# geneo4PETSc/geneo4PETSc

Measured on AMD Instinct MI355X. Metric: GenEO-PCG setup+solve sec and SpMV GB/s, 3D Laplacian 50M DoF, 1/2/4/8 GPUs, higher is better.
Workload: dtype f64

## Files before the change

geneo4petsc_amd/csrc/backend.h:

```cpp
#pragma once
#include <cstddef>
#include <cstdint>

namespace bk {

const char* name();
void set_stream(void* hip_stream);
void* get_stream();
void sync();
void side_stream_begin(void* after = nullptr, bool use_after = false);
void side_stream_end();

int   device_count();
int   set_device(int ordinal);
int   current_device();
int   thread_device_check();
void* alloc(size_t bytes);
void  dfree(void* p);
void  alloc_cache_release();
void  mem_info(double* live, double* live_peak, double* footprint_peak, double* cached, double* dev_free, double* dev_total,
               bool reset_peaks);
void  alloc_stats(double* alloc_s, double* free_s, long long* n);
void  h2d(void* d, const void* h, size_t bytes);
void  d2h(void* h, const void* d, size_t bytes);
// ... 67 lines not shown
void spmv_fused_lp(const Csr& a, int epi, const double* x, double* y, const double* b, double* z, const double* dinv, double w);
bool csr_fusable(const Csr& a);
void spmm_fused(const Csr& a, int epi, const double* X, int ldx, double* Y, int ldy, int m, const double* B, int ldb,
                double* Z, int ldz, const double* dinv, double w);
void csr_diag(const Csr& a, double* diag);
int  recip_positive(double* x, int n);

void gather(double* out, const double* in, const int* idx, int n);
void gather_mul(double* out, const double* in, const int* idx, const double* d, int n);
void segsum(double* out, const double* in, const int* ptr, const int* idx, int nseg, bool accumulate);

void gather_rows(double* out, const double* in, const int* idx, int n, int w);
void segsum_rows(double* out, const double* in, const int* ptr, const int* idx, int nseg, int w, bool accumulate);

void set(double* x, double v, int n);
void copy(double* y, const double* x, int n);
void axpy(double* y, double a, const double* x, int n);
void axpby(double* y, double a, const double* x, double b, int n);
void xmy(double* y, const double* x, const double* d, int n);
void axpy_dev(double* y, const double* a_dev, double sign, const double* x, int n);
void dot(const double* x, const double* y, int n, double* out_dev);

constexpr int CHUNK = 1024;
struct Chunks {
  int nchunk = 0, nsub = 0, n = 0;
  int* start = nullptr;
  int* len = nullptr;
  int* sub = nullptr;
  int* subptr = nullptr;
  int* suboff = nullptr;
  double* partial = nullptr;
  double* totals = nullptr;
  int maxsub_chunks = 0;
};
void set_par_reduce_min(int chunks);
int get_par_reduce_min();
Chunks chunks_upload(int nsub, const int* h_suboff );
void   chunks_free(Chunks& c);
void seg_dot(const Chunks& c, const double* x, const double* y, double* out, int stride, int slot);

void cg_start(const Chunks& c, double* sc, double* x, double* r, double* z, double* p, const double* b,
              const double* dinv);
void seg_pap(const Chunks& c, const double* p, const double* q);
void seg_partial(const Chunks& c, const double* x, const double* y, int slot);
void cg_set_rz(const Chunks& c, double* sc);
void dense_sym_apply(const Chunks& c, const double* inv, const int64_t* base, const double* B, int ldb, double* X,
                     int ldx, int m);
void cg_update(const Chunks& c, double* sc, int parity, double* x, double* r, double* z, const double* p,
               const double* q, const double* dinv);
void cg_direction(const Chunks& c, double* sc, int parity, double* p, const double* z, double tol2);

void gram(const Chunks& c, const double* S, int lds, int p, const double* T, int ldt, int q, double* G);
void gram2(const Chunks& c, const double* S1, int lds1, int p1, const double* S2, int lds2, int p2, const double* T, int ldt,
           int q, double* G);
void block_mul(const Chunks& c, const double* S, int lds, int p, const double* C, int q, double* Y, int ldy,
               bool accumulate);
void block_residual(const Chunks& c, const double* AX, int lda, const double* BX, int ldb, const double* lam,
                    int m, double* R, int ldr, double* nrm);
void block_colnorm(const Chunks& c, const double* X, int ldx, int m, double* nrm);
void block_residual_norms(const Chunks& c, const double* AX, int lda, const double* BX, int ldb, const double* lam,
                          int m, double* R, int ldr, const double* colmask, double* nrm3);
void lobpcg_update32(const Chunks& c, const double* S, const double* AS, const double* BS, const double* C,
                     const double* keep, const double* lam, const double* mask, double* T, double* AT, double* BT,
                     double* R);
void lobpcg_update32_basis(const Chunks& c, const double* S, const double* C, const double* keep, double* T);
bool lobpcg_update32_available();
// ... 43 lines not shown
```

geneo4petsc_amd/csrc/backend_hip.hip:

```cpp
#include <hip/hip_runtime.h>

#include <algorithm>
#include <atomic>
#include <cstdio>
#include <cstdlib>
#include <functional>
#include <stdexcept>
#include <string>
#include <chrono>
#include <condition_variable>
#include <cstring>
#include <thread>
#include <type_traits>
#include <map>
#include <mutex>
#include <unordered_map>
#include <vector>

#include "backend.h"

#define HIPCHK(x)                                                                          \
  do {                                                                                     \
    hipError_t e_ = (x);                                                                   \
    if (e_ != hipSuccess) {                                                                \
      throw std::runtime_error(std::string("HIP error ") + hipGetErrorString(e_) + " at " + \
                               __FILE__ + ":" + std::to_string(__LINE__));                 \
    }                                                                                      \
  } while (0)

namespace bk {

static hipStream_t g_stream_main = nullptr;
static thread_local hipStream_t t_stream_side = nullptr;
static thread_local bool t_side = false;
static thread_local bool g_capturing = false;
static thread_local hipStream_t g_capture_stream = nullptr;
static std::atomic<int> g_device{-1};
static thread_local bool t_dev_bound = false;
static inline void bind_thread() {
  if (t_dev_bound) return;
  t_dev_bound = true;
  const int want = g_device.load(std::memory_order_acquire);
  if (want < 0) {
    int d = 0;
    if (hipGetDevice(&d) == hipSuccess) g_device.store(d, std::memory_order_release);
    else (void)hipGetLastError();
  } else {
    int d = -1;
    if (hipGetDevice(&d) != hipSuccess || d != want) {
      if (hipSetDevice(want) != hipSuccess) throw std::runtime_error("geneo: hipSetDevice failed on a library thread");
    }
  }
// ... 1627 lines not shown
};
template <int EPI>
__device__ __forceinline__ double epi_apply(double sum, double e_b, double e_z, double e_d, double e_x, double w,
                                            double& zout) {
  if (EPI == EPI_NONE) {
    return sum;
  } else if (EPI == EPI_RES) {
    return e_b - sum;
  } else if (EPI == EPI_ADD) {
    return e_z + sum;
  } else if (EPI == EPI_JAC) {
    return e_x + w * e_d * (e_b - sum);
  } else if (EPI == EPI_POST) {
    return w * e_d * (e_z + e_b) + sum;
  } else {
    zout = w * e_d * e_b;
    return e_b - w * sum;
  }
}
struct EpiRow {
  double b = 0.0, z = 0.0, d = 0.0, x = 0.0;
};
template <int EPI>
__device__ __forceinline__ EpiRow epi_load_row(int64_t r, const double* __restrict__ b, const double* __restrict__ z,
                                               const double* __restrict__ dinv, const double* __restrict__ x) {
  EpiRow e;
  if (EpiReads<EPI>::b) e.b = b[r];
  if (EpiReads<EPI>::z) e.z = z[r];
  if (EpiReads<EPI>::d(z)) e.d = dinv[r];
  if (EpiReads<EPI>::x) e.x = x[r];
  return e;
}
template <int EPI>
__device__ __forceinline__ void epi_store_row(int64_t r, double sum, const EpiRow& e, double w, double* __restrict__ y,
                                              double* __restrict__ z) {
  double zv = 0.0;
  const double yv = epi_apply<EPI>(sum, e.b, e.z, e.d, e.x, w, zv);
  if (EPI == EPI_PRE && z) z[r] = zv;
  y[r] = yv;
}

template <bool PAIR_SUM, bool NARROW, bool P16, bool EPI_EARLY>
struct SlicePolicy {
  static constexpr bool pair_sum = PAIR_SUM, narrow = NARROW, p16 = P16, epi_early = EPI_EARLY;
  static_assert(NARROW || !P16, "the predicated form continues the narrow forms");
  static __device__ __forceinline__ double sum4(const double (&acc)[4]) {
    return PAIR_SUM ? (acc[0] + acc[1]) + (acc[2] + acc[3]) : ((acc[0] + acc[1]) + acc[2]) + acc[3];
  }
};
typedef SlicePolicy<false, true, false, true> SliceSell;
typedef SlicePolicy<false, false, false, true> SliceEpi;
typedef SlicePolicy<true, false, false, false> SliceWide;
typedef SlicePolicy<true, true, true, true> SliceLp;

template <int KW, typename VT, int EPI, bool NT, typename POL, typename SRC>
__device__ __forceinline__ double row_sum_fixed(const SRC& src, const VT* __restrict__ val, int64_t e0,
                                                const double* __restrict__ xin, const double* __restrict__ cs) {
  int c[KW];
  double v[KW];
#pragma unroll
  for (int u = 0; u < KW; ++u) {
    c[u] = src.at(u, e0);
    v[u] = (double)(NT ? __builtin_nontemporal_load(val + e0 + 64 * u) : val[e0 + 64 * u]);
  }
  src.template finish<KW>(c);
  double xv[KW];
#pragma unroll
  for (int u = 0; u < KW; ++u) xv[u] = (EPI == EPI_PRE && cs) ? xin[c[u]] * cs[c[u]] : xin[c[u]];
  double acc[4] = {0.0, 0.0, 0.0, 0.0};
  constexpr int NG = KW / 4;
#pragma unroll
  for (int g = 0; g < NG; ++g)
// ... 17 lines not shown
    default: return row_sum_fixed<8, VT, EPI, NT, POL>(src, val, e0, xin, cs);
  }
}
template <int EPI, typename COLT, bool NT>
__device__ __forceinline__ double lp_row_sum_p16(const COLT* __restrict__ col, const float* __restrict__ val, int64_t e0,
                                                 int wd, const int4 cb, const double* __restrict__ xin,
                                                 const double* __restrict__ cs) {
  int c[16];
  double v[16];
#pragma unroll
  for (int u = 0; u < 16; ++u) {
    c[u] = cb.x;
    v[u] = 0.0;
    if (u < wd) {
      c[u] = (u < cb.z ? cb.x : cb.y) + (int)(NT ? __builtin_nontemporal_load(col + e0 + 64 * u) : col[e0 + 64 * u]);
      v[u] = (double)(NT ? __builtin_nontemporal_load(val + e0 + 64 * u) : val[e0 + 64 * u]);
    }
  }
  double xv[16];
#pragma unroll
  for (int u = 0; u < 16; ++u) {
    xv[u] = 0.0;
    if (u < wd) xv[u] = (EPI == EPI_PRE && cs) ? xin[c[u]] * cs[c[u]] : xin[c[u]];
  }
  double acc[4] = {0.0, 0.0, 0.0, 0.0};
  const int ng4 = (wd >> 2) << 2;
#pragma unroll
  for (int u = 0; u < 16; ++u) {
    if (u < ng4) acc[u & 3] += v[u] * xv[u];
    else if (u < wd) acc[0] += v[u] * xv[u];
  }
  return (acc[0] + acc[1]) + (acc[2] + acc[3]);
}
template <typename VT, typename COLT, int EPI, int WPS, bool NT, bool OFFS, typename POL>
__device__ __forceinline__ void spmv_sell_slice(const int64_t* __restrict__ sl_ptr, int nslice, int n,
                                                const COLT* __restrict__ col, const VT* __restrict__ val,
                                                const int* __restrict__ base, const double* __restrict__ x,
                                                double* __restrict__ y, const double* __restrict__ b,
                                                double* __restrict__ z, const double* __restrict__ dinv, double w,
                                                const double* __restrict__ cs ,
                                                const unsigned char* __restrict__ omask, const int* __restrict__ orec) {
  static_assert(WPS == 1 || (WPS == 4 && !OFFS), "a coded slice belongs to one wave");
  constexpr bool FIXED = POL::narrow && WPS == 1;
  const int wv = threadIdx.x >> 6, l = threadIdx.x & 63;
  int s;
  if (WPS == 1) {
    const int nwb = (nslice + 3) >> 2;
    const int t = xcd_remap(blockIdx.x, nwb);
    s = 4 * t + wv;
    if (t >= nwb || s >= nslice) return;
  } else {
    s = xcd_remap(blockIdx.x, nslice);
    if (s >= nslice) return;
  }
  const int su = OFFS ? __builtin_amdgcn_readfirstlane(s) : s;
  const int64_t a = sl_ptr[su], e1 = sl_ptr[su + 1];
  const int4 cb = lp_base_of(base, su);
  int4 o0 = int4{OFF_NONE, 0, 0, 0}, o1 = int4{0, 0, 0, 0};
  int nofix = 0;
  if (OFFS) {
    const int4* rec = reinterpret_cast<const int4*>(orec) + 2 * (int64_t)su;
    o0 = rec[0];
    o1 = rec[1];
    nofix = g_lp_no_fixed;
  }
  const double* __restrict__ xin = (EPI == EPI_PRE) ? b : x;
  const int r = 64 * s + l;
  unsigned char om = 0;
  int oov = 0;
  if (OFFS) {
    om = omask[r];
    oov = orec[8 * (int64_t)su + (l & 7)];
  }
  EpiRow ep;
  if (POL::epi_early && r < n && (WPS == 1 || wv == 0)) ep = epi_load_row<EPI>(r, b, z, dinv, x);
  constexpr int STEP = 64 * WPS;
  double acc[4] = {0.0, 0.0, 0.0, 0.0};
  int64_t e = a + (WPS == 1 ? 0 : 64 * wv) + l;
  int k = (WPS == 1 ? 0 : wv);
  const int wd = (int)((e1 - a) >> 6);
  double fixed_sum = 0.0;
  bool fixed = false;
  if constexpr (FIXED) fixed = wd >= 1 && wd <= (POL::p16 ? 16 : 8) && !(OFFS ? nofix : g_lp_no_fixed);
  if constexpr (FIXED) {
    if (OFFS && fixed && o0.x != OFF_NONE) {
      fixed_sum = row_sum_narrow<VT, EPI, NT, POL>(wd, ColsOffset{o0, o1, om, oov, r, r < n ? r : n - 1}, val, e, xin, cs);
      e = e1;
    } else if (POL::p16 && fixed && wd > 8) {
      if constexpr (POL::p16) fixed_sum = lp_row_sum_p16<EPI, COLT, NT>(col, val, e, wd, cb, xin, cs);
      e = e1;
    } else if (fixed) {
      fixed_sum = row_sum_narrow<VT, EPI, NT, POL>(wd, ColsStored<COLT, NT>{col, cb}, val, e, xin, cs);
      e = e1;
    }
  }
  for (; e + STEP * 3 < e1; e += STEP * 4, k += WPS * 4) {
    int c[4];
    double v[4];
#pragma unroll
    for (int u = 0; u < 4; ++u) {
      c[u] = (k + WPS * u < cb.z ? cb.x : cb.y) + (int)(NT ? __builtin_nontemporal_load(col + e + STEP * u) : col[e + STEP * u]);
      v[u] = (double)(NT ? __builtin_nontemporal_load(val + e + STEP * u) : val[e + STEP * u]);
    }
#pragma unroll
    for (int u = 0; u < 4; ++u) acc[u] += v[u] * ((EPI == EPI_PRE && cs) ? xin[c[u]] * cs[c[u]] : xin[c[u]]);
  }
  for (; e < e1; e += STEP, k += WPS) {
    const int c0 = (k < cb.z ? cb.x : cb.y) + (int)(NT ? __builtin_nontemporal_load(col + e) : col[e]);
    const double v0 = (double)(NT ? __builtin_nontemporal_load(val + e) : val[e]);
    acc[0] += v0 * ((EPI == EPI_PRE && cs) ? xin[c0] * cs[c0] : xin[c0]);
  }
  double sum = fixed ? fixed_sum : POL::sum4(acc);
  if (WPS == 4) {
    __shared__ double part[3][64];
    if (wv > 0) part[wv - 1][l] = sum;
    __syncthreads();
    if (wv > 0) return;
    sum = (sum + part[0][l]) + (part[1][l] + part[2][l]);
  }
  if (r >= n) return;
  if (!POL::epi_early) ep = epi_load_row<EPI>(r, b, z, dinv, x);
  epi_store_row<EPI>(r, sum, ep, w, y, z);
}

template <bool NT, typename COLT = int, bool OFFS = false>
__global__ __launch_bounds__(256) void k_spmv_sell(const int64_t* __restrict__ sl_ptr, int nslice, int n,
                                                   const COLT* __restrict__ col, const double* __restrict__ val,
                                                   const double* __restrict__ x, double* __restrict__ y,
                                                   const int* __restrict__ cbase = nullptr,
                                                   const unsigned char* __restrict__ omask = nullptr,
                                                   const int* __restrict__ orec = nullptr) {
  spmv_sell_slice<double, COLT, EPI_NONE, 1, NT, OFFS, SliceSell>(sl_ptr, nslice, n, col, val, cbase, x, y, nullptr, nullptr,
                                                                  nullptr, 0.0, nullptr, omask, orec);
}
template <bool NT, int EPI>
__global__ __launch_bounds__(256) void k_spmv_sell_epi(const int64_t* __restrict__ sl_ptr, int nslice, int n,
                                                       const int* __restrict__ col, const double* __restrict__ val,
                                                       const double* __restrict__ x, double* __restrict__ y,
                                                       const double* __restrict__ b, double* __restrict__ z,
                                                       const double* __restrict__ dinv, double w,
                                                       const double* __restrict__ cs) {
  spmv_sell_slice<double, int, EPI, 1, NT, false, SliceEpi>(sl_ptr, nslice, n, col, val, nullptr, x, y, b, z, dinv, w, cs,
                                                            nullptr, nullptr);
}
template <int EPI>
__global__ __launch_bounds__(256) void k_spmv_sell_wide(const int64_t* __restrict__ sl_ptr, int nslice, int n,
                                                        const int* __restrict__ col, const double* __restrict__ val,
                                                        const double* __restrict__ x, double* __restrict__ y,
                                                        const double* __restrict__ b, double* __restrict__ z,
                                                        const double* __restrict__ dinv, double w,
                                                        const double* __restrict__ cs) {
// ... 309 lines not shown
    d2h(hstat, dstat, sizeof(hstat));
    dfree(dstat);
    int hfail[2];
    memcpy(hfail, &hstat[0], sizeof(hfail));
    const unsigned long long* hcnt = hstat + 1;
    if (hfail[0]) {
      dfree(a.lp_base);
      a.lp_base = nullptr;
    } else {
      a.lp_col = (unsigned short*)alloc(sizeof(unsigned short) * (size_t)std::max<int64_t>(1, a.sl_nnz));
      a.off_coded = (int)hcnt[0];
      a.off_nnz = (int64_t)hcnt[1];
    }
    const bool off_use = a.lp_col && a.off_coded > 0 && 10 * (int64_t)a.off_coded >= 9 * (int64_t)a.nslice;
    if (!off_use) {
      dfree(a.off_mask);
      dfree(a.off_rec);
      a.off_mask = nullptr;
      a.off_rec = nullptr;
    }
    if (getenv("GENEO_DEBUG"))
      fprintf(stderr, "[offsets] %d-row matrix, %d slices, %d coded%s\n", a.n, a.nslice, a.off_coded,
              !off_try ? " (too wide: not tried)" : off_use ? "" : (a.off_coded ? " (under 90 %: stored columns kept)" : ""));
    if (getenv("GENEO_DEBUG") && (hfail[0] || hfail[1]))
      fprintf(stderr, "[lp] %d-row matrix, %d slices: %s (span limit %d)\n", a.n, a.nslice,
              hfail[0] ? "32-bit columns kept (a slice needs more than two bases)"
                       : (std::to_string(hfail[1]) + " slices with two column bases").c_str(), limit);
  }
  a.lp_val = (float*)alloc(sizeof(float) * (size_t)std::max<int64_t>(1, a.sl_nnz));
  hipLaunchKernelGGL(k_lp_fill, dim3((a.nslice + 3) / 4), dim3(256), 0, g_stream, a.nslice, a.sl_ptr, a.sl_col, a.sl_val,
                     (const int4*)a.lp_base, (index_owner || !a.lp_col) ? (unsigned short*)nullptr : a.lp_col, a.lp_val);
  return true;
}
template <int EPI, int WPS, typename COLT, bool NT, bool OFFS = false>
__global__ __launch_bounds__(256) void k_spmv_sell_lp(const int64_t* __restrict__ sl_ptr, int nslice, int n,
                                                      const COLT* __restrict__ col, const float* __restrict__ val,
                                                      const int* __restrict__ base, const double* __restrict__ x,
                                                      double* __restrict__ y, const double* __restrict__ b,
                                                      double* __restrict__ z, const double* __restrict__ dinv, double w,
                                                      const double* __restrict__ cs,
                                                      const unsigned char* __restrict__ omask = nullptr,
                                                      const int* __restrict__ orec = nullptr) {
  spmv_sell_slice<float, COLT, EPI, WPS, NT, OFFS, SliceLp>(sl_ptr, nslice, n, col, val, base, x, y, b, z, dinv, w, cs, omask,
                                                            orec);
}
struct LpArgs {
  const double* x;
  double* y;
  const double* b;
  double* z;
  const double* dinv;
  double w;
  const double* cs;
};
template <int EPI, int WPS, typename COLT, bool OFFS>
static void spmv_lp_launch_as(const Csr& a, const COLT* col, bool nt, const LpArgs& v) {
  const int grid = 8 * (WPS == 4 ? (a.nslice + 7) / 8 : ((a.nslice + 3) / 4 + 7) / 8);
  const unsigned char* om = OFFS ? a.off_mask : nullptr;
  const int* orec = OFFS ? a.off_rec : nullptr;
  if (nt)
    hipLaunchKernelGGL((k_spmv_sell_lp<EPI, WPS, COLT, true, OFFS>), dim3(grid), dim3(256), 0, g_stream, a.sl_ptr, a.nslice, a.n,
                       col, a.lp_val, a.lp_base, v.x, v.y, v.b, v.z, v.dinv, v.w, v.cs, om, orec);
  else
    hipLaunchKernelGGL((k_spmv_sell_lp<EPI, WPS, COLT, false, OFFS>), dim3(grid), dim3(256), 0, g_stream, a.sl_ptr, a.nslice, a.n,
                       col, a.lp_val, a.lp_base, v.x, v.y, v.b, v.z, v.dinv, v.w, v.cs, om, orec);
}
template <int EPI>
static void spmv_lp_launch(const Csr& a, const double* x, double* y, const double* b, double* z, const double* dinv, double w) {
  if (!a.lp_val) throw std::runtime_error("spmv_lp: the matrix has no single-precision companion");
  if (a.n == 0) return;
  constexpr int nvec = EPI == EPI_NONE ? 2 : (EPI == EPI_POST ? 5 : (EPI == EPI_JAC ? 4 : 3));
  const double ebytes = a.lp_col ? 6.0 : 8.0;
  const bool wide = sell_wide(a);
  const bool offs = g_sell_offsets && a.off_mask && a.off_rec && a.lp_col && !wide;
  const double obytes = offs ? 96.0 * a.off_coded - 2.0 * (double)a.off_nnz : 0.0;
  ProfScope prof(PROF_LP, (double)a.sl_nnz * ebytes >= 32e6,
                 (double)a.sl_nnz * ebytes + obytes + 4.0 * a.nslice + 8.0 * nvec * (double)a.n, 2.0 * (double)a.nnz);
  static const bool nt_off = getenv("GENEO_LP_NO_NT") != nullptr;
  const bool nt = !nt_off && (double)a.sl_nnz * ebytes >= 24e6;
  const LpArgs v{x, y, b, z, dinv, w, (EPI == EPI_PRE && !a.col_scaled) ? dinv : nullptr};
  if (wide) {
    if (a.lp_col) spmv_lp_launch_as<EPI, 4, unsigned short, false>(a, a.lp_col, nt, v);
    else spmv_lp_launch_as<EPI, 4, int, false>(a, a.sl_col, nt, v);
  } else if (offs) {
    spmv_lp_launch_as<EPI, 1, unsigned short, true>(a, a.lp_col, nt, v);
  } else if (a.lp_col) {
    spmv_lp_launch_as<EPI, 1, unsigned short, false>(a, a.lp_col, nt, v);
  } else {
    spmv_lp_launch_as<EPI, 1, int, false>(a, a.sl_col, nt, v);
  }
}
void spmv_lp(const Csr& a, const double* x, double* y) { spmv_lp_launch<EPI_NONE>(a, x, y, nullptr, nullptr, nullptr, 0.0); }
void spmv_fused_lp(const Csr& a, int epi, const double* x, double* y, const double* b, double* z, const double* dinv, double w) {
  switch (epi) {
    case EPI_RES: spmv_lp_launch<EPI_RES>(a, x, y, b, z, dinv, w); break;
    case EPI_ADD: spmv_lp_launch<EPI_ADD>(a, x, y, b, z, dinv, w); break;
    case EPI_JAC: spmv_lp_launch<EPI_JAC>(a, x, y, b, z, dinv, w); break;
    case EPI_POST: spmv_lp_launch<EPI_POST>(a, x, y, b, z, dinv, w); break;
    case EPI_PRE: spmv_lp_launch<EPI_PRE>(a, x, y, b, z, dinv, w); break;
    default: throw std::runtime_error("spmv_fused_lp: unknown epilogue");
  }
}

template <int LPR, int EPI>
__global__ __launch_bounds__(256) void k_spmv_vec(int n, const int* __restrict__ rowptr, const int* __restrict__ col,
                                                  const double* __restrict__ val, const double* __restrict__ x,
                                                  double* __restrict__ y, const double* __restrict__ b,
                                                  double* __restrict__ z, const double* __restrict__ dinv, double w) {
  constexpr int RPB = 256 / LPR;
  const int lane = threadIdx.x % LPR;
  const int64_t r = (int64_t)blockIdx.x * RPB + threadIdx.x / LPR;
  const bool live = r < n;
  double s = 0.0;
  if (live) {
    const int k1 = rowptr[r + 1];
    for (int k = rowptr[r] + lane; k < k1; k += LPR) {
      const int c = col[k];
      s += val[k] * (EPI == EPI_PRE ? b[c] * dinv[c] : x[c]);
    }
  }
#pragma unroll
  for (int o = LPR / 2; o > 0; o >>= 1) s += __shfl_xor(s, o, LPR);
  if (!live || lane != 0) return;
  epi_store_row<EPI>(r, s, epi_load_row<EPI>(r, b, z, dinv, x), w, y, z);
}
template <int EPI>
static void spmv_vec_launch(const Csr& a, const double* x, double* y, const double* b, double* z, const double* dinv,
                            double w) {
#define VEC_LAUNCH(L)                                                                                              \
  hipLaunchKernelGGL((k_spmv_vec<L, EPI>), dim3(grid1d(a.n, 256 / L)), dim3(256), 0, g_stream, a.n, a.rowptr, a.col, \
                     a.val, x, y, b, z, dinv, w)
// ... 844 lines not shown
  int nb = std::min(DOT_BLOCKS, std::max(1, cdiv(n, 2048)));
  hipLaunchKernelGGL(k_dot1, dim3(nb), dim3(256), 0, g_stream, x, y, (int64_t)n, g_dot_work);
  hipLaunchKernelGGL(k_dot2, dim3(1), dim3(256), 0, g_stream, g_dot_work, nb, out_dev);
}

Chunks chunks_upload(int nsub, const int* h_suboff) {
  Chunks c;
  c.nsub = nsub;
  c.n = h_suboff[nsub] - h_suboff[0];
  std::vector<int> st, ln, sb, sp;
  sp.push_back(0);
  for (int s = 0; s < nsub; ++s) {
    for (int a = h_suboff[s]; a < h_suboff[s + 1]; a += CHUNK) {
      st.push_back(a);
      ln.push_back(std::min(CHUNK, h_suboff[s + 1] - a));
      sb.push_back(s);
    }
    c.maxsub_chunks = std::max(c.maxsub_chunks, (int)st.size() - sp.back());
    sp.push_back((int)st.size());
  }
  c.nchunk = (int)st.size();
  c.totals = (double*)alloc(sizeof(double) * 4 * (size_t)std::max(1, nsub));
  c.start = (int*)alloc(sizeof(int) * std::max<size_t>(1, st.size()));
  c.len = (int*)alloc(sizeof(int) * std::max<size_t>(1, st.size()));
  c.sub = (int*)alloc(sizeof(int) * std::max<size_t>(1, st.size()));
  c.subptr = (int*)alloc(sizeof(int) * sp.size());
  c.partial = (double*)alloc(sizeof(double) * 4 * std::max<size_t>(1, st.size()));
  c.suboff = (int*)alloc(sizeof(int) * (size_t)(nsub + 1));
  h2d(c.suboff, h_suboff, sizeof(int) * (size_t)(nsub + 1));
  h2d(c.start, st.data(), sizeof(int) * st.size());
  h2d(c.len, ln.data(), sizeof(int) * ln.size());
  h2d(c.sub, sb.data(), sizeof(int) * sb.size());
  h2d(c.subptr, sp.data(), sizeof(int) * sp.size());
  return c;
}
void gram_plan_drop(const Chunks& c);
void chunks_free(Chunks& c) {
  if (c.start) gram_plan_drop(c);
  dfree(c.start); dfree(c.len); dfree(c.sub); dfree(c.subptr); dfree(c.partial); dfree(c.suboff); dfree(c.totals);
  c = Chunks();
}

__device__ __forceinline__ double sub_total(const double* __restrict__ part, int nchunk, int slot, int c0, int c1) {
  double s = 0.0;
  for (int c = c0; c < c1; ++c) s += part[(int64_t)slot * nchunk + c];
  return s;
}

__device__ __forceinline__ double sub_total_block(const double* __restrict__ part, int nchunk, int slot, int c0,
                                                  int c1, double* sm) {
  double s = 0.0;
  for (int c = c0 + (int)threadIdx.x; c < c1; c += 256) s += part[(int64_t)slot * nchunk + c];
  return block_sum_256(s, sm);
}

static int g_par_reduce_min = getenv("GENEO_PAR_REDUCE_MIN") ? atoi(getenv("GENEO_PAR_REDUCE_MIN")) : 1024;
static inline bool big_subs(const Chunks& c) { return c.maxsub_chunks > g_par_reduce_min; }
void set_par_reduce_min(int chunks) { g_par_reduce_min = chunks; }
int get_par_reduce_min() { return g_par_reduce_min; }
__global__ __launch_bounds__(256) void k_sub_totals(const int* __restrict__ subptr, const double* __restrict__ part,
                                                    int nchunk, int mask, double* __restrict__ totals) {
  __shared__ double sm[4];
  const int s = blockIdx.x, slot = blockIdx.y;
  if (!((mask >> slot) & 1)) return;
  const double t = sub_total_block(part, nchunk, slot, subptr[s], subptr[s + 1], sm);
  if (threadIdx.x == 0) totals[(int64_t)s * 4 + slot] = t;
}
static void sub_totals(const Chunks& c, int mask) {
  hipLaunchKernelGGL(k_sub_totals, dim3(c.nsub, 4), dim3(256), 0, g_stream, c.subptr, c.partial, c.nchunk, mask, c.totals);
}

__global__ __launch_bounds__(256) void k_seg_dot1(const int* __restrict__ start, const int* __restrict__ len,
// ... 71 lines not shown
  q[0] = rz; q[1] = rz; q[2] = 0.0; q[3] = rr; q[4] = 0.0; q[5] = 0.0;
  q[6] = (rr > 0.0) ? 1.0 : 0.0;
  q[7] = rr;
}
void cg_start(const Chunks& c, double* sc, double* x, double* r, double* z, double* p, const double* b,
              const double* dinv) {
  if (c.nchunk == 0) return;
  hipLaunchKernelGGL(k_cg_start, dim3(c.nchunk), dim3(256), 0, g_stream, c.start, c.len, x, r, z, p, b, dinv,
                     c.partial, c.nchunk);
  const bool big = big_subs(c);
  if (big) sub_totals(c, 6);
  hipLaunchKernelGGL(k_cg_start2, dim3(grid1d(c.nsub, 64)), dim3(64), 0, g_stream, c.subptr, c.partial, c.nchunk,
                     sc, c.nsub, big ? c.totals : (const double*)nullptr);
}
void seg_partial(const Chunks& c, const double* x, const double* y, int slot) {
  if (c.nchunk == 0) return;
  hipLaunchKernelGGL(k_seg_dot1, dim3(c.nchunk), dim3(256), 0, g_stream, c.start, c.len, x, y, c.partial, c.nchunk,
                     slot);
}
__global__ void k_cg_start3(const int* __restrict__ subptr, const double* __restrict__ part, int nchunk,
                            double* __restrict__ sc, int nsub, const double* __restrict__ totals) {
  int s = blockIdx.x * blockDim.x + threadIdx.x;
  if (s >= nsub) return;
  const double rz = totals ? totals[(int64_t)s * 4 + 1] : sub_total(part, nchunk, 1, subptr[s], subptr[s + 1]);
  sc[(int64_t)s * 8 + 0] = rz;
  sc[(int64_t)s * 8 + 1] = rz;
}
void cg_set_rz(const Chunks& c, double* sc) {
  if (c.nchunk == 0) return;
  const bool big = big_subs(c);
  if (big) sub_totals(c, 2);
  hipLaunchKernelGGL(k_cg_start3, dim3(grid1d(c.nsub, 64)), dim3(64), 0, g_stream, c.subptr, c.partial, c.nchunk, sc,
                     c.nsub, big ? c.totals : (const double*)nullptr);
}
void seg_pap(const Chunks& c, const double* p, const double* q) {
  if (c.nchunk == 0) return;
  hipLaunchKernelGGL(k_seg_dot1, dim3(c.nchunk), dim3(256), 0, g_stream, c.start, c.len, p, q, c.partial,
                     c.nchunk, 0);
}
__global__ __launch_bounds__(256) void k_cg_update(const int* __restrict__ start, const int* __restrict__ len,
                                                   const int* __restrict__ sub, const int* __restrict__ subptr,
                                                   double* __restrict__ sc, int parity, double* __restrict__ x,
                                                   double* __restrict__ r, double* __restrict__ z,
                                                   const double* __restrict__ p, const double* __restrict__ q,
                                                   const double* __restrict__ dinv, double* __restrict__ part,
                                                   int nchunk, const double* __restrict__ totals) {
  __shared__ double sm[4];
  const int c = blockIdx.x;
  const int s = sub[c];
  const int c0 = subptr[s], c1 = subptr[s + 1];
  const double pap = totals ? totals[(int64_t)s * 4 + 0] : sub_total_block(part, nchunk, 0, c0, c1, sm);
  const double rz = sc[(int64_t)s * 8 + parity];
  const double active = sc[(int64_t)s * 8 + 6];
  const double alpha = (active != 0.0 && pap != 0.0) ? rz / pap : 0.0;
  const int a = start[c], n = len[c];
  double nrz = 0.0, nrr = 0.0;
  for (int i = threadIdx.x; i < n; i += 256) {
    const double xv = x[a + i] + alpha * p[a + i];
    const double rv = r[a + i] - alpha * q[a + i];
    x[a + i] = xv;
    r[a + i] = rv;
    if (dinv) {
      const double zv = dinv[a + i] * rv;
      z[a + i] = zv;
      nrz += rv * zv;
    }
// ... 27 lines not shown
  __shared__ double sm[4];
  const int c = blockIdx.x;
  const int s = sub[c];
  const int c0 = subptr[s], c1 = subptr[s + 1];
  const double nrz = totals ? totals[(int64_t)s * 4 + 1] : sub_total_block(part, nchunk, 1, c0, c1, sm);
  const double nrr = totals ? totals[(int64_t)s * 4 + 2] : sub_total_block(part, nchunk, 2, c0, c1, sm);
  const double rz = sc[(int64_t)s * 8 + parity];
  const double was_active = sc[(int64_t)s * 8 + 6];
  const double rr0 = sc[(int64_t)s * 8 + 7];
  const double beta = (was_active != 0.0 && rz != 0.0) ? nrz / rz : 0.0;
  const int a = start[c], n = len[c];
  if (was_active != 0.0) {
    for (int i = threadIdx.x; i < n; i += 256) p[a + i] = z[a + i] + beta * p[a + i];
  }
  if (threadIdx.x == 0 && c == c0) {
    sc[(int64_t)s * 8 + (parity ^ 1)] = nrz;
    sc[(int64_t)s * 8 + 3] = nrr;
    sc[(int64_t)s * 8 + 5] = beta;
  }
  (void)tol2; (void)rr0;
}
__global__ void k_cg_flag(double* __restrict__ sc, double tol2, int nsub) {
  int s = blockIdx.x * blockDim.x + threadIdx.x;
  if (s >= nsub) return;
  double* q = sc + (int64_t)s * 8;
  if (q[6] != 0.0 && q[3] <= tol2 * q[7]) q[6] = 0.0;
}
void cg_direction(const Chunks& c, double* sc, int parity, double* p, const double* z, double tol2) {
  if (c.nchunk == 0) return;
  const bool big = big_subs(c);
  if (big) sub_totals(c, 6);
  hipLaunchKernelGGL(k_cg_direction, dim3(c.nchunk), dim3(256), 0, g_stream, c.start, c.len, c.sub, c.subptr, sc,
                     parity, p, z, tol2, c.partial, c.nchunk, big ? c.totals : (const double*)nullptr);
  hipLaunchKernelGGL(k_cg_flag, dim3(grid1d(c.nsub, 64)), dim3(64), 0, g_stream, sc, tol2, c.nsub);
}

constexpr int GRAM_CH = 1;

using d4 = __attribute__((ext_vector_type(4))) double;

template <int TI, int TJ, int NC>
__global__ __launch_bounds__(256) __attribute__((amdgpu_waves_per_eu(3))) void k_gram_mfma(const int* __restrict__ cstart, const int* __restrict__ clen,
                                                   const int* __restrict__ gfirst, const int* __restrict__ gcount,
                                                   const double* __restrict__ S, int lds_, int p,
                                                   const double* __restrict__ T, int ldt_, int q,
                                                   double* __restrict__ Gpart, int I0, int J0,
                                                   const double* __restrict__ S2, int lds2_, int psplit) {
  extern __shared__ __attribute__((aligned(16))) double smem[];
  const int ldS = (p % 32 == 0) ? p + 16 : p;
  const int ldT = (q % 32 == 0) ? q + 16 : q;
  double* sS = smem;
  double* sT = smem + 16 * ldS;
  const int g = blockIdx.x;
  const int c0 = gfirst[g], nc = gcount[g];
  const int row0 = cstart[c0];
  int nrows = 0;
  for (int c = 0; c < nc; ++c) nrows += clen[c0 + c];
  const int tid = threadIdx.x, w = tid >> 6, l = tid & 63;
  const int P16 = p >> 4, Q16 = q >> 4;
  const int wi = w >> 1, wj = w & 1;
  int aoff[TI], boff[TJ];
#pragma unroll
  for (int a = 0; a < TI; ++a) {
    int I = I0 + wi * TI + a;
    if (I >= P16) I = P16 - 1;
    aoff[a] = 16 * I + (l & 15);
// ... 1167 lines not shown
```

geneo4petsc_amd/csrc/capi.cpp:

```cpp
#include <dlfcn.h>

#include <cstdio>
#include <cstdlib>
#include <cstring>
#include <exception>
#include <stdexcept>
#include <string>
#include <vector>

#include <algorithm>
#include <chrono>
#include <thread>

#include "../../include/geneo_c.h"
#include "coarse_dev.h"
#include "core.h"
#include "dense.h"

struct _p_GeneoPC {
  geneo::PC* ctx = nullptr;
  std::string name, err, optstr;
  bool has_ops = false;
  int nbDOF = 0, nbDOFLoc = 0;
  std::vector<int> map, rowptr, col;
  std::vector<double> val;
  const double* b_dev = nullptr;
};

struct _p_GeneoSpmv {
  bk::Csr a;
};

static std::string g_global_err;

#define GUARD_BEGIN try {
#define GUARD_END(pc)                                \
  }                                                  \
  catch (std::exception & e) {                       \
    if (pc) (pc)->err = e.what();                    \
    else g_global_err = e.what();                    \
    return 1;                                        \
  }

static int pcfail(PC pc, const std::string& m) {
  if (pc) pc->err = m;
  return 1;
}
static int propagate(PC pc, int rc) {
  if (rc && pc && pc->ctx) pc->err = pc->ctx->last_error;
// ... 945 lines not shown
                                double* sc_out) {
  if (!h) return 1;
  GUARD_BEGIN
  const int n = suboff[nsub], n0 = suboff[0];
  bk::Chunks c = bk::chunks_upload(nsub, suboff);
  double* sc = (double*)bk::alloc(sizeof(double) * 8 * (size_t)std::max(1, nsub));
  double* q = (double*)bk::alloc(sizeof(double) * (size_t)std::max(1, n));
  const double* dv = caller_precond ? nullptr : dinv;
  bk::cg_start(c, sc, x, r, z, p, b, dv);
  if (caller_precond) {
    bk::xmy(z + n0, r + n0, dinv + n0, n - n0);
    bk::seg_partial(c, r, z, 1);
    bk::cg_set_rz(c, sc);
    bk::copy(p + n0, z + n0, n - n0);
  }
  int parity = 0;
  for (int it = 0; it < iters; ++it) {
    bk::spmv(h->a, p, q);
    bk::seg_pap(c, p, q);
    bk::cg_update(c, sc, parity, x, r, z, p, q, dv);
    if (caller_precond) {
      bk::xmy(z + n0, r + n0, dinv + n0, n - n0);
      bk::seg_partial(c, r, z, 1);
    }
    bk::cg_direction(c, sc, parity, p, z, tol2);
    parity ^= 1;
  }
  bk::d2h(sc_out, sc, sizeof(double) * 8 * (size_t)nsub);
  bk::dfree(sc);
  bk::dfree(q);
  bk::chunks_free(c);
  GUARD_END((PC) nullptr)
  return 0;
}

long long GeneoTestCsrOp(int op, const GeneoCsr* A, const GeneoCsr* B, const int* iarg, const double* darg,
                         void* const* parg, int* rowptr_out, int* col_out, double* val_out, long long cap) {
  try {
    const bool layouts = (op == 0 || op == 1);
    bk::Csr a = layouts ? bk::csr_upload(A->n, A->rowptr, A->col, A->val) : bk::csr_upload_raw(A->n, A->rowptr, A->col, A->val);
    bk::Csr b, c;
    long long nnz = -2;
    auto out = [&](const bk::Csr& m) {
      nnz = (long long)m.nnz;
      if (cap >= nnz && rowptr_out) bk::csr_download(m, rowptr_out, col_out, val_out);
    };
    if (op == 0) {
      c = bk::csr_remap_columns(a, (const int*)parg[0]);
      out(c);
      bk::csr_free(c);
    } else if (op == 1) {
      c = bk::csr_scaled_alias(a, (const double*)parg[0], (const double*)parg[1], iarg[0] != 0);
      if (iarg[1] > 0)
        bk::spmm_fused(c, bk::EPI_PRE, nullptr, 0, (double*)parg[2], iarg[2], iarg[1], (const double*)parg[3], iarg[3],
                       (double*)parg[4], iarg[4], (const double*)parg[5], darg[0]);
      out(c);
      bk::csr_free(c);
    } else if (op == 2) {
      b = bk::csr_tentative_prolongator(A->n, (const int*)parg[0]);
      if (iarg[1]) {
        bool ok = true;
        c = bk::spgemm(a, b, iarg[0], &ok);
        if (ok) {
          bk::smooth_prolongator(c, (const int*)parg[0], (const double*)parg[1], darg[0]);
          out(c);
          bk::csr_free(c);
// ... 34 lines not shown
```

geneo4petsc_amd/csrc/core.cpp:

```cpp
#include "core.h"

#include <algorithm>
#include <atomic>
#include <chrono>
#include <cfloat>
#include <cmath>
#include <cstdio>
#include <cstdlib>
#include <cstring>
#include <condition_variable>
#include <exception>
#include <mutex>
#include <functional>
#include <future>
#include <map>
#include <numeric>
#include <fstream>
#include <iomanip>
#include <sstream>
#include <stdexcept>
#include <thread>

#include "amg.h"
#include "coarse_dev.h"
#include "dense.h"

namespace bk {
__attribute__((weak)) bool coarse_factor(const double*, int, int, double*, double*, int*) { return false; }
__attribute__((weak)) bool coarse_solve(const double*, const double*, int, int, double*) { return false; }
}

namespace geneo {

// ... 999 lines not shown
  if (size == 1) {
    bk::segsum_rows(Y, WL, d_rt_ptr, d_rt_idx, nown, w, false);
    return;
  }
  bk::segsum_rows(ye, WL, d_rt_ptr, d_rt_idx, nE, w, false);
  bk::copy(comm_send, ye + (int64_t)nown * w, (int)((int64_t)nH * w));
  if (cb_exchange(cb_user, 1 | (w << 1))) throw std::runtime_error("GenEO: halo exchange callback failed");
  bk::copy(Y, ye, (int)((int64_t)nown * w));
  bk::segsum_rows(Y, comm_recv, d_rv_ptr, d_rv_idx, nown, w, true);
}

void PC::matmult_block(const double* X, double* Y, int w, double* WL, double* xe) {
  info.spmv_calls += w;
  if (size == 1) {
    bk::spmm_strided(neuE, X, w, WL, w, w, nullptr, nullptr);
  } else {
    const int nown = n_owned();
    bk::gather_rows(comm_send, X, d_send_idx, (int)send_idx.size(), w);
    if (cb_exchange(cb_user, 0 | (w << 1))) throw std::runtime_error("GenEO: halo exchange callback failed");
    bk::copy(xe, X, (int)((int64_t)nown * w));
    bk::copy(xe + (int64_t)nown * w, comm_recv, (int)((int64_t)nH * w));
    bk::spmm_strided(neuE, xe, w, WL, w, w, nullptr, nullptr);
  }
  prolong_block(WL, Y, w, xe);
}

void PC::local_solve(double* wL) {
  if (opt.lvl1RAS) bk::xmy(wL, wL, d_D, nL);
  const int ns = (int)subs.size();
  const bool use_amg = (opt.dls1_pc == "amg") && amg1;
  double* x = d_xL;
  const double* dinv = use_amg ? nullptr : d_dinv1;
  bk::cg_start(ch, d_cg_sc, x, d_cg_r, d_cg_z, d_cg_p, wL, dinv);
  if (use_amg) {
    amg1->vcycle(d_cg_r, 1, d_cg_z, 1, 1);
    bk::seg_partial(ch, d_cg_r, d_cg_z, 1);
    bk::cg_set_rz(ch, d_cg_sc);
    bk::copy(d_cg_p, d_cg_z, nL);
  }
  const double tol2 = opt.dls1_rtol * opt.dls1_rtol;
  std::vector<double> sc((size_t)8 * std::max(1, ns));
  int it = 0;
  int parity = 0;
  static const int amg_check = getenv("GENEO_DLS1_AMG_CHECK") ? atoi(getenv("GENEO_DLS1_AMG_CHECK")) : 4;
  const int check = std::max(1, use_amg ? std::min(amg_check, opt.dls1_check) : opt.dls1_check);
  bool done = false;
  auto chunk = [&](int len) {
    for (int k = 0; k < len; ++k) {
      bk::spmv(dirL, d_cg_p, d_cg_q);
      bk::seg_pap(ch, d_cg_p, d_cg_q);
      bk::cg_update(ch, d_cg_sc, parity, x, d_cg_r, d_cg_z, d_cg_p, d_cg_q, dinv);
      if (use_amg) {
        amg1->vcycle(d_cg_r, 1, d_cg_z, 1, 1);
        bk::seg_partial(ch, d_cg_r, d_cg_z, 1);
      }
      bk::cg_direction(ch, d_cg_sc, parity, d_cg_p, d_cg_z, tol2);
      parity ^= 1;
    }
  };
  auto graph_for = [&](int len) -> void* {
    if ((len % 2 != 0 && len != 1) || cg_graph_failed) return nullptr;
    const int key = 2 * len + parity;
    auto it_g = cg_graphs.find(key);
    if (it_g != cg_graphs.end()) return it_g->second;
    void* g = nullptr;
    const int parity_in = parity;
    if (bk::graph_capture_begin()) {
      try {
        chunk(len);
      } catch (...) {
        bk::graph_capture_end();
        cg_graph_failed = true;
        throw;
      }
      g = bk::graph_capture_end();
      parity = parity_in;
    }
    if (!g) cg_graph_failed = true;
    else cg_graphs[key] = g;
    return g;
  };
  static const bool dbg_dls1 = getenv("GENEO_DEBUG_DLS1") != nullptr;
  std::vector<int> conv_at(dbg_dls1 ? ns : 0, -1);
  auto run = [&](int len) {
    void* g = graph_for(len);
    const bool direct = !g || (bk::spmv_profiling() && (cg_chunks++ % 8 == 0));
    if (!direct) {
      bk::graph_launch(g);
      parity ^= (len & 1);
    } else {
      chunk(len);
    }
    it += len;
    bk::d2h(sc.data(), d_cg_sc, sizeof(double) * 8 * ns);
    done = true;
// ... 2080 lines not shown
```

Measured before the change: 6458.

## Fuse the r·z dot product into the V-cycle's final post-smoothing SpMV

```diff
diff --git a/geneo4petsc_amd/csrc/backend.h b/geneo4petsc_amd/csrc/backend.h
--- a/geneo4petsc_amd/csrc/backend.h
+++ b/geneo4petsc_amd/csrc/backend.h
@@ -123,6 +123,9 @@
   double* partial = nullptr;
   double* totals = nullptr;
   int maxsub_chunks = 0;
+  int* slice_split = nullptr;
+  double* slice_part = nullptr;
+  int nslice64 = 0;
 };
 void set_par_reduce_min(int chunks);
 int get_par_reduce_min();
diff --git a/geneo4petsc_amd/csrc/backend_dots.h b/geneo4petsc_amd/csrc/backend_dots.h
--- /dev/null
+++ b/geneo4petsc_amd/csrc/backend_dots.h
@@ -0,0 +1,12 @@
+#pragma once
+#include "backend.h"
+
+namespace bk {
+
+#define GENEO_BK_OPTIONAL __attribute__((weak))
+GENEO_BK_OPTIONAL void post_rz_expect(const Chunks& c, const double* r);
+GENEO_BK_OPTIONAL bool post_rz_taken();
+GENEO_BK_OPTIONAL void cg_set_rz_dots(const Chunks& c, double* sc);
+GENEO_BK_OPTIONAL void cg_direction_dots(const Chunks& c, double* sc, int parity, double* p, const double* z, double tol2);
+
+}
diff --git a/geneo4petsc_amd/csrc/backend_hip.hip b/geneo4petsc_amd/csrc/backend_hip.hip
--- a/geneo4petsc_amd/csrc/backend_hip.hip
+++ b/geneo4petsc_amd/csrc/backend_hip.hip
@@ -18,6 +18,7 @@
 #include <vector>
 
 #include "backend.h"
+#include "backend_dots.h"
 
 #define HIPCHK(x)                                                                          \
   do {                                                                                     \
@@ -1711,12 +1712,13 @@
   return e;
 }
 template <int EPI>
-__device__ __forceinline__ void epi_store_row(int64_t r, double sum, const EpiRow& e, double w, double* __restrict__ y,
-                                              double* __restrict__ z) {
+__device__ __forceinline__ double epi_store_row(int64_t r, double sum, const EpiRow& e, double w, double* __restrict__ y,
+                                                double* __restrict__ z) {
   double zv = 0.0;
   const double yv = epi_apply<EPI>(sum, e.b, e.z, e.d, e.x, w, zv);
   if (EPI == EPI_PRE && z) z[r] = zv;
   y[r] = yv;
+  return yv;
 }
 
 template <bool PAIR_SUM, bool NARROW, bool P16, bool EPI_EARLY>
@@ -1800,15 +1802,18 @@
   }
   return (acc[0] + acc[1]) + (acc[2] + acc[3]);
 }
-template <typename VT, typename COLT, int EPI, int WPS, bool NT, bool OFFS, typename POL>
+template <typename VT, typename COLT, int EPI, int WPS, bool NT, bool OFFS, typename POL, bool DOT = false>
 __device__ __forceinline__ void spmv_sell_slice(const int64_t* __restrict__ sl_ptr, int nslice, int n,
                                                 const COLT* __restrict__ col, const VT* __restrict__ val,
                                                 const int* __restrict__ base, const double* __restrict__ x,
                                                 double* __restrict__ y, const double* __restrict__ b,
                                                 double* __restrict__ z, const double* __restrict__ dinv, double w,
                                                 const double* __restrict__ cs ,
-                                                const unsigned char* __restrict__ omask, const int* __restrict__ orec) {
+                                                const unsigned char* __restrict__ omask, const int* __restrict__ orec,
+                                                const int* __restrict__ dsplit = nullptr,
+                                                double* __restrict__ dpart = nullptr) {
   static_assert(WPS == 1 || (WPS == 4 && !OFFS), "a coded slice belongs to one wave");
+  static_assert(!DOT || (WPS == 1 && POL::epi_early && EPI == EPI_POST), "the dot epilogue: wave-per-slice, early operand loads, r.z");
   constexpr bool FIXED = POL::narrow && WPS == 1;
   const int wv = threadIdx.x >> 6, l = threadIdx.x & 63;
   int s;
@@ -1821,9 +1826,11 @@
     s = xcd_remap(blockIdx.x, nslice);
     if (s >= nslice) return;
   }
-  const int su = OFFS ? __builtin_amdgcn_readfirstlane(s) : s;
+  const int su = (OFFS || DOT) ? __builtin_amdgcn_readfirstlane(s) : s;
   const int64_t a = sl_ptr[su], e1 = sl_ptr[su + 1];
   const int4 cb = lp_base_of(base, su);
+  int split = 0;
+  if constexpr (DOT) split = dsplit[su];
   int4 o0 = int4{OFF_NONE, 0, 0, 0}, o1 = int4{0, 0, 0, 0};
   int nofix = 0;
   if (OFFS) {
@@ -1885,6 +1892,16 @@
     __syncthreads();
     if (wv > 0) return;
     sum = (sum + part[0][l]) + (part[1][l] + part[2][l]);
+  }
+  if constexpr (DOT) {
+    double t = 0.0;
+    if (r < n) t = ep.z * epi_store_row<EPI>(r, sum, ep, w, y, z);
+    const bool lo = r < split;
+    const double d0 = wave_sum(lo ? t : 0.0);
+    double d1 = 0.0;
+    if (split < 64 * (su + 1)) d1 = wave_sum(lo ? 0.0 : t);
+    if ((threadIdx.x & 63) == 0) *reinterpret_cast<double2*>(dpart + 2 * (int64_t)su) = double2{d0, d1};
+    return;
   }
   if (r >= n) return;
   if (!POL::epi_early) ep = epi_load_row<EPI>(r, b, z, dinv, x);
@@ -2260,7 +2277,7 @@
                      (const int4*)a.lp_base, (index_owner || !a.lp_col) ? (unsigned short*)nullptr : a.lp_col, a.lp_val);
   return true;
 }
-template <int EPI, int WPS, typename COLT, bool NT, bool OFFS = false>
+template <int EPI, int WPS, typename COLT, bool NT, bool OFFS = false, bool DOT = false>
 __global__ __launch_bounds__(256) void k_spmv_sell_lp(const int64_t* __restrict__ sl_ptr, int nslice, int n,
                                                       const COLT* __restrict__ col, const float* __restrict__ val,
                                                       const int* __restrict__ base, const double* __restrict__ x,
@@ -2268,10 +2285,54 @@
                                                       double* __restrict__ z, const double* __restrict__ dinv, double w,
                                                       const double* __restrict__ cs,
                                                       const unsigned char* __restrict__ omask = nullptr,
-                                                      const int* __restrict__ orec = nullptr) {
-  spmv_sell_slice<float, COLT, EPI, WPS, NT, OFFS, SliceLp>(sl_ptr, nslice, n, col, val, base, x, y, b, z, dinv, w, cs, omask,
-                                                            orec);
-}
+                                                      const int* __restrict__ orec = nullptr,
+                                                      const int* __restrict__ dsplit = nullptr,
+                                                      double* __restrict__ dpart = nullptr) {
+  spmv_sell_slice<float, COLT, EPI, WPS, NT, OFFS, SliceLp, DOT>(sl_ptr, nslice, n, col, val, base, x, y, b, z, dinv, w, cs,
+                                                                 omask, orec, dsplit, dpart);
+}
+__global__ __launch_bounds__(256) void k_slice_totals(const int* __restrict__ suboff, const double* __restrict__ part,
+                                                      int slot, double* __restrict__ totals) {
+  __shared__ double sm[4];
+  const int s = blockIdx.x;
+  const int r0 = suboff[s], r1 = suboff[s + 1];
+  const int jf = (r0 + 63) >> 6, jl = (r1 - 1) >> 6;
+  double t = (threadIdx.x == 0 && (r0 & 63)) ? part[2 * (int64_t)(jf - 1) + 1] : 0.0;
+  for (int j0 = jf + (int)threadIdx.x; j0 <= jl; j0 += 256 * 16) {
+    double v[16];
+#pragma unroll
+    for (int u = 0; u < 16; ++u) {
+      const int j = j0 + 256 * u;
+      v[u] = j <= jl ? part[2 * (int64_t)j] : 0.0;
+    }
+#pragma unroll
+    for (int u = 0; u < 16; ++u) t += v[u];
+  }
+  t = block_sum_256(t, sm);
+  if (threadIdx.x == 0) totals[(int64_t)s * 4 + slot] = t;
+}
+static void slice_totals(const Chunks& c, int slot) {
+  hipLaunchKernelGGL(k_slice_totals, dim3(c.nsub), dim3(256), 0, g_stream, c.suboff, c.slice_part, slot, c.totals);
+}
+static inline bool dots_cover(const Csr& a, const Chunks& c) {
+  return c.slice_split && c.nslice64 > 0 && a.n == c.n && a.nslice == c.nslice64 && a.nlong == 0 && a.vec_lpr == 0;
+}
+static thread_local const Chunks* t_rz_chunks = nullptr;
+static thread_local const double* t_rz_r = nullptr;
+static thread_local bool t_rz_taken = false;
+void post_rz_expect(const Chunks& c, const double* r) {
+  t_rz_chunks = c.slice_split ? &c : nullptr;
+  t_rz_r = r;
+  t_rz_taken = false;
+}
+bool post_rz_taken() {
+  const bool taken = t_rz_taken;
+  t_rz_chunks = nullptr;
+  t_rz_r = nullptr;
+  t_rz_taken = false;
+  return taken;
+}
+
 struct LpArgs {
   const double* x;
   double* y;
@@ -2282,10 +2343,24 @@
   const double* cs;
 };
 template <int EPI, int WPS, typename COLT, bool OFFS>
-static void spmv_lp_launch_as(const Csr& a, const COLT* col, bool nt, const LpArgs& v) {
+static void spmv_lp_launch_as(const Csr& a, const COLT* col, bool nt, const LpArgs& v, const Chunks* dots = nullptr) {
   const int grid = 8 * (WPS == 4 ? (a.nslice + 7) / 8 : ((a.nslice + 3) / 4 + 7) / 8);
   const unsigned char* om = OFFS ? a.off_mask : nullptr;
   const int* orec = OFFS ? a.off_rec : nullptr;
+  if constexpr (EPI == EPI_POST && WPS == 1) {
+    if (dots) {
+      double* part = dots->slice_part;
+      if (nt)
+        hipLaunchKernelGGL((k_spmv_sell_lp<EPI, 1, COLT, true, OFFS, true>), dim3(grid), dim3(256), 0, g_stream, a.sl_ptr,
+                           a.nslice, a.n, col, a.lp_val, a.lp_base, v.x, v.y, v.b, v.z, v.dinv, v.w, v.cs, om, orec,
+                           dots->slice_split, part);
+      else
+        hipLaunchKernelGGL((k_spmv_sell_lp<EPI, 1, COLT, false, OFFS, true>), dim3(grid), dim3(256), 0, g_stream, a.sl_ptr,
+                           a.nslice, a.n, col, a.lp_val, a.lp_base, v.x, v.y, v.b, v.z, v.dinv, v.w, v.cs, om, orec,
+                           dots->slice_split, part);
+      return;
+    }
+  }
   if (nt)
     hipLaunchKernelGGL((k_spmv_sell_lp<EPI, WPS, COLT, true, OFFS>), dim3(grid), dim3(256), 0, g_stream, a.sl_ptr, a.nslice, a.n,
                        col, a.lp_val, a.lp_base, v.x, v.y, v.b, v.z, v.dinv, v.w, v.cs, om, orec);
@@ -2294,7 +2369,8 @@
                        col, a.lp_val, a.lp_base, v.x, v.y, v.b, v.z, v.dinv, v.w, v.cs, om, orec);
 }
 template <int EPI>
-static void spmv_lp_launch(const Csr& a, const double* x, double* y, const double* b, double* z, const double* dinv, double w) {
+static void spmv_lp_launch(const Csr& a, const double* x, double* y, const double* b, double* z, const double* dinv, double w,
+                           const Chunks* dots = nullptr) {
   if (!a.lp_val) throw std::runtime_error("spmv_lp: the matrix has no single-precision companion");
   if (a.n == 0) return;
   constexpr int nvec = EPI == EPI_NONE ? 2 : (EPI == EPI_POST ? 5 : (EPI == EPI_JAC ? 4 : 3));
@@ -2311,11 +2387,11 @@
     if (a.lp_col) spmv_lp_launch_as<EPI, 4, unsigned short, false>(a, a.lp_col, nt, v);
     else spmv_lp_launch_as<EPI, 4, int, false>(a, a.sl_col, nt, v);
   } else if (offs) {
-    spmv_lp_launch_as<EPI, 1, unsigned short, true>(a, a.lp_col, nt, v);
+    spmv_lp_launch_as<EPI, 1, unsigned short, true>(a, a.lp_col, nt, v, dots);
   } else if (a.lp_col) {
-    spmv_lp_launch_as<EPI, 1, unsigned short, false>(a, a.lp_col, nt, v);
+    spmv_lp_launch_as<EPI, 1, unsigned short, false>(a, a.lp_col, nt, v, dots);
   } else {
-    spmv_lp_launch_as<EPI, 1, int, false>(a, a.sl_col, nt, v);
+    spmv_lp_launch_as<EPI, 1, int, false>(a, a.sl_col, nt, v, dots);
   }
 }
 void spmv_lp(const Csr& a, const double* x, double* y) { spmv_lp_launch<EPI_NONE>(a, x, y, nullptr, nullptr, nullptr, 0.0); }
@@ -2324,7 +2400,17 @@
     case EPI_RES: spmv_lp_launch<EPI_RES>(a, x, y, b, z, dinv, w); break;
     case EPI_ADD: spmv_lp_launch<EPI_ADD>(a, x, y, b, z, dinv, w); break;
     case EPI_JAC: spmv_lp_launch<EPI_JAC>(a, x, y, b, z, dinv, w); break;
-    case EPI_POST: spmv_lp_launch<EPI_POST>(a, x, y, b, z, dinv, w); break;
+    case EPI_POST: {
+      const Chunks* dots = (t_rz_chunks && z == t_rz_r && a.n > 0 && a.lp_val && dots_cover(a, *t_rz_chunks) && !sell_wide(a))
+                               ? t_rz_chunks : nullptr;
+      spmv_lp_launch<EPI_POST>(a, x, y, b, z, dinv, w, dots);
+      if (dots) {
+        slice_totals(*dots, 1);
+        t_rz_taken = true;
+        t_rz_chunks = nullptr;
+      }
+      break;
+    }
     case EPI_PRE: spmv_lp_launch<EPI_PRE>(a, x, y, b, z, dinv, w); break;
     default: throw std::runtime_error("spmv_fused_lp: unknown epilogue");
   }
@@ -3235,12 +3321,24 @@
   h2d(c.len, ln.data(), sizeof(int) * ln.size());
   h2d(c.sub, sb.data(), sizeof(int) * sb.size());
   h2d(c.subptr, sp.data(), sizeof(int) * sp.size());
+  bool slices = nsub > 0 && h_suboff[0] == 0 && c.n > 0;
+  for (int s = 0; s < nsub && slices; ++s) slices = h_suboff[s + 1] - h_suboff[s] >= 64;
+  if (slices) {
+    c.nslice64 = (c.n + 63) / 64;
+    std::vector<int> split((size_t)c.nslice64);
+    for (int s = 0, j = 0; s < nsub; ++s)
+      for (; j < c.nslice64 && 64 * (int64_t)j < h_suboff[s + 1]; ++j) split[j] = h_suboff[s + 1];
+    c.slice_split = (int*)alloc(sizeof(int) * split.size());
+    c.slice_part = (double*)alloc(sizeof(double) * 2 * split.size());
+    h2d(c.slice_split, split.data(), sizeof(int) * split.size());
+  }
   return c;
 }
 void gram_plan_drop(const Chunks& c);
 void chunks_free(Chunks& c) {
   if (c.start) gram_plan_drop(c);
   dfree(c.start); dfree(c.len); dfree(c.sub); dfree(c.subptr); dfree(c.partial); dfree(c.suboff); dfree(c.totals);
+  dfree(c.slice_split); dfree(c.slice_part);
   c = Chunks();
 }
 
@@ -3378,6 +3476,11 @@
   if (big) sub_totals(c, 2);
   hipLaunchKernelGGL(k_cg_start3, dim3(grid1d(c.nsub, 64)), dim3(64), 0, g_stream, c.subptr, c.partial, c.nchunk, sc,
                      c.nsub, big ? c.totals : (const double*)nullptr);
+}
+void cg_set_rz_dots(const Chunks& c, double* sc) {
+  if (c.nchunk == 0) return;
+  hipLaunchKernelGGL(k_cg_start3, dim3(grid1d(c.nsub, 64)), dim3(64), 0, g_stream, c.subptr, c.partial, c.nchunk, sc,
+                     c.nsub, (const double*)c.totals);
 }
 void seg_pap(const Chunks& c, const double* p, const double* q) {
   if (c.nchunk == 0) return;
@@ -3471,6 +3574,13 @@
   if (big) sub_totals(c, 6);
   hipLaunchKernelGGL(k_cg_direction, dim3(c.nchunk), dim3(256), 0, g_stream, c.start, c.len, c.sub, c.subptr, sc,
                      parity, p, z, tol2, c.partial, c.nchunk, big ? c.totals : (const double*)nullptr);
+  hipLaunchKernelGGL(k_cg_flag, dim3(grid1d(c.nsub, 64)), dim3(64), 0, g_stream, sc, tol2, c.nsub);
+}
+void cg_direction_dots(const Chunks& c, double* sc, int parity, double* p, const double* z, double tol2) {
+  if (c.nchunk == 0) return;
+  sub_totals(c, 4);
+  hipLaunchKernelGGL(k_cg_direction, dim3(c.nchunk), dim3(256), 0, g_stream, c.start, c.len, c.sub, c.subptr, sc,
+                     parity, p, z, tol2, c.partial, c.nchunk, (const double*)c.totals);
   hipLaunchKernelGGL(k_cg_flag, dim3(grid1d(c.nsub, 64)), dim3(64), 0, g_stream, sc, tol2, c.nsub);
 }
 
diff --git a/geneo4petsc_amd/csrc/capi.cpp b/geneo4petsc_amd/csrc/capi.cpp
--- a/geneo4petsc_amd/csrc/capi.cpp
+++ b/geneo4petsc_amd/csrc/capi.cpp
@@ -15,6 +15,7 @@
 #include "../../include/geneo_c.h"
 #include "coarse_dev.h"
 #include "core.h"
+#include "backend_dots.h"
 #include "dense.h"
 
 struct _p_GeneoPC {
@@ -1026,6 +1027,76 @@
   bk::chunks_free(c);
   GUARD_END((PC) nullptr)
   return 0;
+}
+
+int GeneoTestFusedDots(GeneoSpmv h, int nsub, const int* suboff, int unfused, int iters, double tol2, double w, double* p,
+                       double* q, const double* e, double* r1, double* r, double* z, double* x, const double* b,
+                       const double* dinv, double* totals_out, double* sc_out) {
+  if (!h) return -1;
+  try {
+    if (!bk::csr_has_lp(h->a) && !bk::csr_make_lp(h->a)) throw std::runtime_error("no single-precision companion for this matrix");
+    const int n = suboff[nsub];
+    bk::Chunks c = bk::chunks_upload(nsub, suboff);
+    const bool dots = !unfused && &bk::post_rz_expect != nullptr && c.slice_split != nullptr;
+    auto post = [&](bool want) {
+      if (want) bk::post_rz_expect(c, r);
+      bk::spmv_fused_lp(h->a, bk::EPI_POST, e, z, r1, r, dinv, w);
+      return want && bk::post_rz_taken();
+    };
+    int ran = dots ? 1 : 0;
+    if (iters == 0) {
+      double* t = (double*)bk::alloc(sizeof(double) * 2 * (size_t)std::max(1, nsub));
+      std::vector<double> tot((size_t)4 * std::max(1, nsub));
+      bk::spmv(h->a, p, q);
+      if (dots && !post(true)) ran = 0;
+      if (ran) bk::d2h(tot.data(), c.totals, sizeof(double) * 4 * (size_t)nsub);
+      else post(false);
+      bk::seg_dot(c, p, q, t, 2, 0);
+      bk::seg_dot(c, r, z, t, 2, 1);
+      bk::d2h(totals_out, t, sizeof(double) * 2 * (size_t)nsub);
+      for (int s = 0; s < nsub && ran; ++s) totals_out[2 * s + 1] = tot[4 * (size_t)s + 1];
+      bk::dfree(t);
+    } else {
+      double* sc = (double*)bk::alloc(sizeof(double) * 8 * (size_t)std::max(1, nsub));
+      auto cycle = [&](bool want) {
+        bk::spmv_fused_lp(h->a, bk::EPI_PRE, nullptr, r1, r, nullptr, dinv, w);
+        return post(want);
+      };
+      bk::cg_start(c, sc, x, r, z, p, b, nullptr);
+      if (dots) {
+        if (!cycle(true)) throw std::runtime_error("the EPI_POST pass did not take the r.z epilogue");
+        bk::cg_set_rz_dots(c, sc);
+      } else {
+        cycle(false);
+        bk::seg_partial(c, r, z, 1);
+        bk::cg_set_rz(c, sc);
+      }
+      bk::copy(p, z, n);
+      int parity = 0;
+      for (int it = 0; it < iters; ++it) {
+        bk::spmv(h->a, p, q);
+        bk::seg_pap(c, p, q);
+        bk::cg_update(c, sc, parity, x, r, z, p, q, nullptr);
+        if (dots) {
+          if (!cycle(true)) throw std::runtime_error("the EPI_POST pass did not take the r.z epilogue");
+          bk::cg_direction_dots(c, sc, parity, p, z, tol2);
+        } else {
+          cycle(false);
+          bk::seg_partial(c, r, z, 1);
+          bk::cg_direction(c, sc, parity, p, z, tol2);
+        }
+        parity ^= 1;
+      }
+      bk::d2h(sc_out, sc, sizeof(double) * 8 * (size_t)nsub);
+      bk::dfree(sc);
+    }
+    bk::sync();
+    bk::chunks_free(c);
+    return ran;
+  } catch (std::exception& ex) {
+    g_global_err = ex.what();
+    return -1;
+  }
 }
 
 long long GeneoTestCsrOp(int op, const GeneoCsr* A, const GeneoCsr* B, const int* iarg, const double* darg,
diff --git a/geneo4petsc_amd/csrc/core.cpp b/geneo4petsc_amd/csrc/core.cpp
--- a/geneo4petsc_amd/csrc/core.cpp
+++ b/geneo4petsc_amd/csrc/core.cpp
@@ -1,4 +1,5 @@
 #include "core.h"
+#include "backend_dots.h"
 
 #include <algorithm>
 #include <atomic>
@@ -1064,10 +1065,19 @@
   double* x = d_xL;
   const double* dinv = use_amg ? nullptr : d_dinv1;
   bk::cg_start(ch, d_cg_sc, x, d_cg_r, d_cg_z, d_cg_p, wL, dinv);
+  static const bool fused_dots_on = !(getenv("GENEO_CG_FUSED_DOTS") && atoi(getenv("GENEO_CG_FUSED_DOTS")) == 0);
+  bool dots = false;
   if (use_amg) {
+    const bool try_dots = fused_dots_on && &bk::post_rz_expect != nullptr && ch.slice_split != nullptr;
+    if (try_dots) bk::post_rz_expect(ch, d_cg_r);
     amg1->vcycle(d_cg_r, 1, d_cg_z, 1, 1);
-    bk::seg_partial(ch, d_cg_r, d_cg_z, 1);
-    bk::cg_set_rz(ch, d_cg_sc);
+    dots = try_dots && bk::post_rz_taken();
+    if (dots) {
+      bk::cg_set_rz_dots(ch, d_cg_sc);
+    } else {
+      bk::seg_partial(ch, d_cg_r, d_cg_z, 1);
+      bk::cg_set_rz(ch, d_cg_sc);
+    }
     bk::copy(d_cg_p, d_cg_z, nL);
   }
   const double tol2 = opt.dls1_rtol * opt.dls1_rtol;
@@ -1078,7 +1088,17 @@
   const int check = std::max(1, use_amg ? std::min(amg_check, opt.dls1_check) : opt.dls1_check);
   bool done = false;
   auto chunk = [&](int len) {
-    for (int k = 0; k < len; ++k) {
+    for (int k = 0; k < len && dots; ++k) {
+      bk::spmv(dirL, d_cg_p, d_cg_q);
+      bk::seg_pap(ch, d_cg_p, d_cg_q);
+      bk::cg_update(ch, d_cg_sc, parity, x, d_cg_r, d_cg_z, d_cg_p, d_cg_q, dinv);
+      bk::post_rz_expect(ch, d_cg_r);
+      amg1->vcycle(d_cg_r, 1, d_cg_z, 1, 1);
+      if (!bk::post_rz_taken()) throw std::runtime_error("GenEO: the V-cycle's last pass did not take the r.z epilogue");
+      bk::cg_direction_dots(ch, d_cg_sc, parity, d_cg_p, d_cg_z, tol2);
+      parity ^= 1;
+    }
+    for (int k = 0; k < len && !dots; ++k) {
       bk::spmv(dirL, d_cg_p, d_cg_q);
       bk::seg_pap(ch, d_cg_p, d_cg_q);
       bk::cg_update(ch, d_cg_sc, parity, x, d_cg_r, d_cg_z, d_cg_p, d_cg_q, dinv);
@@ -1092,7 +1112,7 @@
   };
   auto graph_for = [&](int len) -> void* {
     if ((len % 2 != 0 && len != 1) || cg_graph_failed) return nullptr;
-    const int key = 2 * len + parity;
+    const int key = 2 * len + parity + (dots ? (1 << 30) : 0);
     auto it_g = cg_graphs.find(key);
     if (it_g != cg_graphs.end()) return it_g->second;
     void* g = nullptr;
```

Result: slower. 6343 (-1.8%).
